# zhaohanjin/hbbft

Hardware: AMD Instinct MI355X
Metric: verified BLS12-381 shares/sec (whole node) at N=1000; combines/sec (higher is better)
Workload: dtype u32 (381-bit Montgomery limbs); 1 GPU; C3 HoneyBadger epoch: 1000 ciphertexts x 1000 DecryptionShares verified + 1000 G1 combines (t=334); N=1000, f=333, t=334, ciphertexts=1000, parallelism=1 GPU

## Files before the change

### hbbft_amd/csrc/curve.h

```cpp
#pragma once
#include "field.h"

namespace hbtc {

HD void fadd(Fq& r, const Fq& a, const Fq& b) { fq_add(r, a, b); }
HD void fadd(Fq2& r, const Fq2& a, const Fq2& b) { fq2_add(r, a, b); }
HD void fsub(Fq& r, const Fq& a, const Fq& b) { fq_sub(r, a, b); }
HD void fsub(Fq2& r, const Fq2& a, const Fq2& b) { fq2_sub(r, a, b); }
HD void fmul(Fq& r, const Fq& a, const Fq& b) { fq_mul(r, a, b); }
HD void fmul(Fq2& r, const Fq2& a, const Fq2& b) { fq2_mul(r, a, b); }
HD void fsqr(Fq& r, const Fq& a) { fq_sqr(r, a); }
HD void fsqr(Fq2& r, const Fq2& a) { fq2_sqr(r, a); }
HD void fdbl(Fq& r, const Fq& a) { fq_dbl(r, a); }
HD void fdbl(Fq2& r, const Fq2& a) { fq2_dbl(r, a); }
HD void fneg(Fq& r, const Fq& a) { fq_neg(r, a); }
HD void fneg(Fq2& r, const Fq2& a) { fq2_neg(r, a); }
HD bool fis_zero(const Fq& a) { return fq_is_zero(a); }
HD bool fis_zero(const Fq2& a) { return fq2_is_zero(a); }
HD bool feq(const Fq& a, const Fq& b) { return fq_eq(a, b); }
HD bool feq(const Fq2& a, const Fq2& b) { return fq2_eq(a, b); }
HD void fone(Fq& r) { fq_one(r); }
HD void fone(Fq2& r) { fq2_one(r); }
HD void fzero(Fq& r) { fq_zero(r); }
HD void fzero(Fq2& r) { fq2_zero(r); }
// ... 1128 lines not shown
    return;
  }
  fw_mul(u1, p.x, z2z2);
  fw_mul(u2, q.x, z1z1);
  fw_mul(s1, p.y, q.z);
  fw_mul(s1, s1, z2z2);
  fw_mul(s2, q.y, p.z);
  fw_mul(s2, s2, z1z1);
  fw_sub(H, u2, u1, rr::RR_SUB_1_4, 4);
  fw_norm(H, H);
  fw_sub(rr0, s2, s1, rr::RR_SUB_1_4, 4);
  fw_norm(rr0, rr0);
  fw_sqr(HH, H);
  if (fw_is_zero(HH)) {
    fw_one(t);
    fw_mul(t, rr0, t);
    if (fw_is_zero(t)) {
      jacw_dbl(r, p);
    } else {
      jacw_set_inf(r);
    }
    return;
  }
  fw_add(t, p.z, q.z);
  fw_norm(t, t);
  fw_sqr(z3, t);
  fw_add(t, z1z1, z2z2);
  fw_sub(z3, z3, t, rr::RR_SUB_2_4, 4);
  fw_norm(z3, z3);
  fw_mul(z3, z3, H);
  jacw_add_tail(r, u1, s1, H, HH, rr0, z3);
}
HD bool jacw_eq_aff(const JacW& p, const FqW& ax, const FqW& ay) {
  FqW z2, z3, t, u, one;
  fw_one(one);
  fw_sqr(z2, p.z);
  fw_mul(z3, z2, p.z);
  fw_mul(t, ax, z2);
  fw_mul(u, p.x, one);
  if (!fw_eq(t, u)) return false;
  fw_mul(t, ay, z3);
  fw_mul(u, p.y, one);
  return fw_eq(t, u);
}
HDN void jacw_mul_x(JacW& r, const AffW& q) {
  JacW acc;
  jacw_set_inf(acc);
  for (int b = 63; b >= 0; --b) {
    jacw_dbl(acc, acc);
    if ((BLS_X_ABS >> b) & 1ull) jacw_add_aff(acc, acc, q);
  }
  r = acc;
}
HDN void jacw_mul_x_jac(JacW& r, const JacW& q) {
  JacW acc;
  jacw_set_inf(acc);
  for (int b = 63; b >= 0; --b) {
    jacw_dbl(acc, acc);
    if ((BLS_X_ABS >> b) & 1ull) jacw_add(acc, acc, q);
  }
  r = acc;
}
HDN bool g1_in_subgroup_t1_w(const G1A& p, G1J& t) {
  if (p.inf) {
    jac_set_inf(t);
    return true;
  }
  AffW q;
  affw_from_aff(q, p);
  JacW t1, t2;
  jacw_mul_x(t1, q);
  jacw_to_jac(t, t1);
  jacw_mul_x_jac(t2, t1);
  if (jacw_is_inf(t2)) return false;
  FqW beta, bx, ny;
  Fq fb;
  fq_set(fb, G1_BETA);
  fw_from_fq(beta, fb);
  fw_mul(bx, q.x, beta);
  fw_neg(ny, q.y);
  return jacw_eq_aff(t2, bx, ny);
}

HD void g2_psi(Fq2& rx, Fq2& ry, const G2A& p) {
  Fq2 c, k;
  fq2_conj(c, p.x);
  fq2_set(k, G2_PSI_CX);
  fq2_mul(rx, c, k);
  fq2_conj(c, p.y);
  fq2_set(k, G2_PSI_CY);
  fq2_mul(ry, c, k);
}

HDN bool g2_in_subgroup(const G2A& p) {
  if (p.inf) return true;
  G2J t;
  jac_mul_u64(t, p, BLS_X_ABS);
  if (jac_is_inf(t)) return false;
  Fq2 px, py, npy;
  g2_psi(px, py, p);
  fq2_neg(npy, py);
  return jac_eq_aff(t, px, npy);
}

HD void g2j_psi(G2J& r, const G2J& p) {
  Fq2 c, k;
  fq2_conj(c, p.x);
  fq2_set(k, G2_PSI_CX);
  fq2_mul(r.x, c, k);
  fq2_conj(c, p.y);
  fq2_set(k, G2_PSI_CY);
  fq2_mul(r.y, c, k);
  fq2_conj(r.z, p.z);
}

HD uint32_t cofactor_c0_word(int i) {
  return i == 0 ? G2_CLEAR_C0[0] : i == 1 ? G2_CLEAR_C0[1] : i == 2 ? G2_CLEAR_C0[2] : G2_CLEAR_C0[3];
}
HDN void g2_clear_cofactor(G2J& out, const G2A& p) {
  if (p.inf) {
    jac_set_inf(out);
    return;
  }
  G2J pj, t1, t2, t3;
  jac_from_aff(pj, p);
  jac_mul_u64(t1, p, BLS_X_ABS);
  jac_neg(t1, t1);
  G2A ps;
  g2_psi(ps.x, ps.y, p);
  ps.inf = 0;
  jac_dbl(t3, pj);
  g2j_psi(t3, t3);
  g2j_psi(t3, t3);
  {
    G2A nps;
    aff_neg(nps, ps);
    jac_add_aff(t3, t3, nps);
  }
  jac_add_aff(t2, t1, ps);
  jac_mul_u64_jac(t2, t2, BLS_X_ABS);
  jac_neg(t2, t2);
  jac_add(t3, t3, t2);
  {
    G2J nt1;
    jac_neg(nt1, t1);
    jac_add(t3, t3, nt1);
  }
  {
    G2A np;
    aff_neg(np, p);
    jac_add_aff(t3, t3, np);
  }
  if (jac_is_inf(t3)) {
    out = t3;
    return;
  }
  G2J mq = t3;
  {
    Fq zeta;
    fq_set(zeta, G2_ZETA);
    fq_mul(mq.x.c0, t3.x.c0, zeta);
    fq_mul(mq.x.c1, t3.x.c1, zeta);
  }
  G2J bj;
  jac_add(bj, t3, mq);
  G2A b;
// ... 184 lines not shown
```

### hbbft_amd/csrc/field.h

```cpp
#pragma once
#include <cstdint>

#if defined(__HIPCC__) || defined(__HIP__)
#include <hip/hip_runtime.h>
#define HD __host__ __device__ __forceinline__
#if defined(HBTC_INLINE_ALL)
#define HDN __host__ __device__ __forceinline__
#else
#define HDN __host__ __device__ inline __attribute__((noinline))
#endif
#define HBTC_CONST static constexpr
#ifndef HBTC_LATENCY_PRIO_LEVEL
#define HBTC_LATENCY_PRIO_LEVEL 2
#endif
#if defined(__HIP_DEVICE_COMPILE__)
#define HBTC_LATENCY_PRIO() __builtin_amdgcn_s_setprio(HBTC_LATENCY_PRIO_LEVEL)
#else
#define HBTC_LATENCY_PRIO() ((void)0)
#endif
#else
#define HD static inline
#define HDN static inline __attribute__((noinline))
#define HBTC_CONST static constexpr
#endif

#include "bls_constants.h"
#include "fq_fips.h"
#ifndef HBTC_FIPS_ONEBLOCK
#define HBTC_FIPS_ONEBLOCK 1
#endif
#if HBTC_FIPS_ONEBLOCK
#include "fq_fips_asm.h"
#endif
#if defined(HBTC_FQMUL_SR)
#include "fq_fips_sr.h"
#endif
#ifndef HBTC_FQ_RR
#define HBTC_FQ_RR 2
#endif
#include "fq_rr.h"

#ifndef HBTC_FQ_UNROLL
#define HBTC_FQ_UNROLL 1
#endif

#define HBTC_PRAGMA(x) _Pragma(#x)
#define HBTC_UNROLL_N(n) HBTC_PRAGMA(unroll n)

namespace hbtc {

template <int N>
struct Limbs {
  uint32_t v[N];
};

typedef Limbs<12> Fq;
typedef Limbs<8> Fr;

HD uint32_t addc32(uint32_t a, uint32_t b, uint32_t cin, uint32_t* cout) {
  return __builtin_addc(a, b, cin, cout);
}
HD uint32_t subb32(uint32_t a, uint32_t b, uint32_t bin, uint32_t* bout) {
  return __builtin_subc(a, b, bin, bout);
}

template <int N>
HD uint32_t limbs_add(Limbs<N>& r, const Limbs<N>& a, const Limbs<N>& b) {
  uint32_t c = 0;
#pragma unroll
  for (int i = 0; i < N; ++i) r.v[i] = addc32(a.v[i], b.v[i], c, &c);
  return c;
}

template <int N>
HD uint32_t limbs_sub(Limbs<N>& r, const Limbs<N>& a, const Limbs<N>& b) {
  uint32_t c = 0;
#pragma unroll
  for (int i = 0; i < N; ++i) r.v[i] = subb32(a.v[i], b.v[i], c, &c);
  return c;
}

template <int N>
HD uint32_t limbs_sub_const(Limbs<N>& r, const Limbs<N>& a, const uint32_t* m) {
  uint32_t c = 0;
#pragma unroll
  for (int i = 0; i < N; ++i) r.v[i] = subb32(a.v[i], m[i], c, &c);
  return c;
}

template <int N>
HD uint32_t limbs_add_const(Limbs<N>& r, const Limbs<N>& a, const uint32_t* m) {
  uint32_t c = 0;
#pragma unroll
  for (int i = 0; i < N; ++i) r.v[i] = addc32(a.v[i], m[i], c, &c);
  return c;
}

template <int N>
HD void limbs_select(Limbs<N>& r, bool take_b, const Limbs<N>& a, const Limbs<N>& b) {
#pragma unroll
  for (int i = 0; i < N; ++i) r.v[i] = take_b ? b.v[i] : a.v[i];
}

template <int N>
HD bool limbs_is_zero(const Limbs<N>& a) {
  uint32_t acc = 0;
#pragma unroll
  for (int i = 0; i < N; ++i) acc |= a.v[i];
  return acc == 0;
}

template <int N>
HD bool limbs_eq(const Limbs<N>& a, const Limbs<N>& b) {
  uint32_t acc = 0;
#pragma unroll
  for (int i = 0; i < N; ++i) acc |= a.v[i] ^ b.v[i];
  return acc == 0;
}

template <int N>
HD bool limbs_lt_const(const Limbs<N>& a, const uint32_t* m) {
// ... 654 lines not shown
}
HD void fw_sqr(FqW& r, const FqW& a) {
#if HBTC_FW_TRACK
  fw_check_operand(a);
  const uint64_t vb = fw_prod_vb(a.vb, a.vb);
#endif
#if defined(__HIP_DEVICE_COMPILE__)
  rr::mont_sqr_w_asm(r.v, a.v);
#else
  rr::mont_sqr_w_cxx(r.v, a.v);
#endif
#if HBTC_FW_TRACK
  fw_set_strict(r, vb);
#endif
}
HD void fw_set(FqW& r, const uint32_t (&c)[13]) {
#pragma unroll
  for (int i = 0; i < 13; ++i) r.v[i] = c[i];
#if HBTC_FW_TRACK
  fw_set_strict(r, FW_ONE_P);
#endif
}
HD void fw_one(FqW& r) { fw_set(r, rr::RR_ONE); }
HD void fw_zero(FqW& r) {
#pragma unroll
  for (int i = 0; i < 13; ++i) r.v[i] = 0;
#if HBTC_FW_TRACK
  uint64_t lb[13] = {0};
  fw_set_bounds(r, lb, 0);
#endif
}
HD void fw_neg(FqW& r, const FqW& a) {
  FqW z;
  fw_zero(z);
  fw_sub(r, z, a, rr::RR_SUB_1_4, 4);
  fw_norm(r, r);
}
HD bool fw_is_zero(const FqW& a) {
#if HBTC_FW_TRACK
  for (int i = 0; i < 12; ++i)
    if (a.lb[i] > rr::RR_MASK) fw_fail("zero test on limbs above 2^30 - 1");
  if (a.vb >= 2 * FW_ONE_P) fw_fail("zero test on a value that may reach 2p");
#endif
  uint32_t z = 0, d = 0;
#pragma unroll
  for (int i = 0; i < 13; ++i) {
    z |= a.v[i];
    d |= a.v[i] ^ rr::RR_P[i];
  }
  return z == 0 || d == 0;
}
HD bool fw_eq(const FqW& a, const FqW& b) {
#if HBTC_FW_TRACK
  for (int i = 0; i < 12; ++i)
    if (a.lb[i] > rr::RR_MASK || b.lb[i] > rr::RR_MASK) fw_fail("comparison on limbs above 2^30 - 1");
  if (a.vb >= 2 * FW_ONE_P || b.vb >= 2 * FW_ONE_P) fw_fail("comparison of a value that may reach 2p");
#endif
  FqR x, y;
#pragma unroll
  for (int i = 0; i < 13; ++i) {
    x.v[i] = a.v[i];
    y.v[i] = b.v[i];
  }
  return fqr_eq(x, y);
}
HD void fw_from_fq(FqW& r, const Fq& a) {
  FqR t;
  fqr_from_fq(t, a);
#pragma unroll
  for (int i = 0; i < 13; ++i) r.v[i] = t.v[i];
#if HBTC_FW_TRACK
  fw_set_strict(r, FW_ONE_P + FW_ONE_P / 2);
#endif
}
HD void fw_to_fq(Fq& r, const FqW& a) {
  FqW k, t;
  fw_set(k, rr::RR_K_OUT);
  fw_mul(t, a, k);
  FqR u;
#pragma unroll
  for (int i = 0; i < 13; ++i) u.v[i] = t.v[i];
  fqr_limbs32(r, u);
}

HD bool fq_is_lex_largest(const Fq& a) {
  Fq c;
  fq_from_mont(c, a);
  Fq t;
  uint32_t borrow = limbs_sub_const<12>(t, c, P_MINUS_1_DIV_2);
  return borrow == 0 && !limbs_is_zero<12>(t);
}

HD void fr_canon(Fr& r, const Fr& a) {
  Fr t;
  uint32_t borrow = limbs_sub_const<8>(t, a, FR_R);
  limbs_select<8>(r, borrow == 0, a, t);
}

HD void fr_mul(Fr& r, const Fr& a, const Fr& b) {
  Fr t;
  mont_mul<8, 8>(t, a, b, FR_R, FR_NP);
  fr_canon(r, t);
}

HD void fr_add(Fr& r, const Fr& a, const Fr& b) {
  limbs_add<8>(r, a, b);
  fr_canon(r, r);
}

HD void fr_sub(Fr& r, const Fr& a, const Fr& b) {
  uint32_t borrow = limbs_sub<8>(r, a, b);
  Fr t;
  limbs_add_const<8>(t, r, FR_R);
  limbs_select<8>(r, borrow != 0, r, t);
}

HD void fr_to_mont(Fr& r, const Fr& a) {
  Fr r2;
  limbs_set_const<8>(r2, FR_R2);
  fr_mul(r, a, r2);
  fr_canon(r, r);
}

HD void fr_from_mont(Fr& r, const Fr& a) {
  Fr one;
  limbs_zero<8>(one);
  one.v[0] = 1;
  fr_mul(r, a, one);
  fr_canon(r, r);
}

HDN void fr_pow_const(Fr& r, const Fr& a, const uint32_t* e) {
  Fr acc;
  limbs_set_const<8>(acc, FR_ONE);
  for (int w = 7; w >= 0; --w) {
    const uint32_t word = e[w];
    for (int b = 31; b >= 0; --b) {
      fr_mul(acc, acc, acc);
      if ((word >> b) & 1u) fr_mul(acc, acc, a);
    }
  }
  fr_canon(r, acc);
}

HD void fr_inv(Fr& r, const Fr& a) { fr_pow_const(r, a, EXP_R_MINUS_2); }

HD void fr_from_u64(Fr& r, uint64_t x) {
  Fr a;
  limbs_zero<8>(a);
  a.v[0] = (uint32_t)x;
  a.v[1] = (uint32_t)(x >> 32);
  fr_to_mont(r, a);
}

struct Fq2 {
  Fq c0, c1;
};

HD void fq2_zero(Fq2& r) {
  fq_zero(r.c0);
  fq_zero(r.c1);
}
HD void fq2_one(Fq2& r) {
  fq_one(r.c0);
  fq_zero(r.c1);
}
// ... 405 lines not shown
```

### hbbft_amd/csrc/fq_rr.h

```cpp
#pragma once
#include <cstdint>
#if defined(__HIPCC__) || defined(__HIP__)
#define HBTC_RR_HD __host__ __device__ __forceinline__
#else
#define HBTC_RR_HD static inline
#endif
#define HBTC_RR_CONST static constexpr
#if defined(HBTC_RR_ASSERT) && !defined(__HIP_DEVICE_COMPILE__)
#include <cstdio>
#include <cstdlib>
#define HBTC_RR_MAD(acc, x, y)                                                          \
  do {                                                                                  \
    if (__builtin_add_overflow((acc), (uint64_t)(x) * (y), &(acc))) {                   \
      std::fprintf(stderr, "fq_rr: MAD carry-out at %s:%d\n", __FILE__, __LINE__);       \
      std::abort();                                                                     \
    }                                                                                   \
  } while (0)
#else
#define HBTC_RR_MAD(acc, x, y) ((acc) += (uint64_t)(x) * (y))
#endif
namespace hbtc {
namespace rr {

HBTC_RR_CONST uint32_t RR_P[13] = {0x3fffaaabu, 0x27fbffffu, 0x153ffffbu, 0x2affffacu, 0x30f6241eu, 0x034a83dau, 0x112bf673u, 0x12e13ce1u, 0x2cd76477u, 0x1ed90d2eu, 0x29a4b1bau, 0x3a8e5ff9u, 0x001a0111u};
// ... 1502 lines not shown
      "v_mad_u64_u32 v[" HBTC_XS(HBTC_FIPS_ACC2) ":" HBTC_XS(HBTC_FIPS_ACC3) "], vcc, %23, %59, v[" HBTC_XS(HBTC_FIPS_ACC2) ":" HBTC_XS(HBTC_FIPS_ACC3) "]\n\t"
      "v_mad_u64_u32 v[" HBTC_XS(HBTC_FIPS_ACC2) ":" HBTC_XS(HBTC_FIPS_ACC3) "], vcc, %24, %58, v[" HBTC_XS(HBTC_FIPS_ACC2) ":" HBTC_XS(HBTC_FIPS_ACC3) "]\n\t"
      "v_mad_u64_u32 v[" HBTC_XS(HBTC_FIPS_ACC2) ":" HBTC_XS(HBTC_FIPS_ACC3) "], vcc, %25, %57, v[" HBTC_XS(HBTC_FIPS_ACC2) ":" HBTC_XS(HBTC_FIPS_ACC3) "]\n\t"
      "v_and_b32 %4, %66, v" HBTC_XS(HBTC_FIPS_ACC2) "\n\t"
      "v_alignbit_b32 v" HBTC_XS(HBTC_FIPS_ACC0) ", v" HBTC_XS(HBTC_FIPS_ACC3) ", v" HBTC_XS(HBTC_FIPS_ACC2) ", 30\n\t"
      "v_lshrrev_b32 v" HBTC_XS(HBTC_FIPS_ACC1) ", 30, v" HBTC_XS(HBTC_FIPS_ACC3) "\n\t"
      "v_mad_u64_u32 v[" HBTC_XS(HBTC_FIPS_ACC0) ":" HBTC_XS(HBTC_FIPS_ACC1) "], vcc, %33, %51, v[" HBTC_XS(HBTC_FIPS_ACC0) ":" HBTC_XS(HBTC_FIPS_ACC1) "]\n\t"
      "v_mad_u64_u32 v[" HBTC_XS(HBTC_FIPS_ACC0) ":" HBTC_XS(HBTC_FIPS_ACC1) "], vcc, %34, %50, v[" HBTC_XS(HBTC_FIPS_ACC0) ":" HBTC_XS(HBTC_FIPS_ACC1) "]\n\t"
      "v_mad_u64_u32 v[" HBTC_XS(HBTC_FIPS_ACC0) ":" HBTC_XS(HBTC_FIPS_ACC1) "], vcc, %35, %49, v[" HBTC_XS(HBTC_FIPS_ACC0) ":" HBTC_XS(HBTC_FIPS_ACC1) "]\n\t"
      "v_mad_u64_u32 v[" HBTC_XS(HBTC_FIPS_ACC0) ":" HBTC_XS(HBTC_FIPS_ACC1) "], vcc, %36, %36, v[" HBTC_XS(HBTC_FIPS_ACC0) ":" HBTC_XS(HBTC_FIPS_ACC1) "]\n\t"
      "v_mad_u64_u32 v[" HBTC_XS(HBTC_FIPS_ACC0) ":" HBTC_XS(HBTC_FIPS_ACC1) "], vcc, %19, %64, v[" HBTC_XS(HBTC_FIPS_ACC0) ":" HBTC_XS(HBTC_FIPS_ACC1) "]\n\t"
      "v_mad_u64_u32 v[" HBTC_XS(HBTC_FIPS_ACC0) ":" HBTC_XS(HBTC_FIPS_ACC1) "], vcc, %20, %63, v[" HBTC_XS(HBTC_FIPS_ACC0) ":" HBTC_XS(HBTC_FIPS_ACC1) "]\n\t"
      "v_mad_u64_u32 v[" HBTC_XS(HBTC_FIPS_ACC0) ":" HBTC_XS(HBTC_FIPS_ACC1) "], vcc, %21, %62, v[" HBTC_XS(HBTC_FIPS_ACC0) ":" HBTC_XS(HBTC_FIPS_ACC1) "]\n\t"
      "v_mad_u64_u32 v[" HBTC_XS(HBTC_FIPS_ACC0) ":" HBTC_XS(HBTC_FIPS_ACC1) "], vcc, %22, %61, v[" HBTC_XS(HBTC_FIPS_ACC0) ":" HBTC_XS(HBTC_FIPS_ACC1) "]\n\t"
      "v_mad_u64_u32 v[" HBTC_XS(HBTC_FIPS_ACC0) ":" HBTC_XS(HBTC_FIPS_ACC1) "], vcc, %23, %60, v[" HBTC_XS(HBTC_FIPS_ACC0) ":" HBTC_XS(HBTC_FIPS_ACC1) "]\n\t"
      "v_mad_u64_u32 v[" HBTC_XS(HBTC_FIPS_ACC0) ":" HBTC_XS(HBTC_FIPS_ACC1) "], vcc, %24, %59, v[" HBTC_XS(HBTC_FIPS_ACC0) ":" HBTC_XS(HBTC_FIPS_ACC1) "]\n\t"
      "v_mad_u64_u32 v[" HBTC_XS(HBTC_FIPS_ACC0) ":" HBTC_XS(HBTC_FIPS_ACC1) "], vcc, %25, %58, v[" HBTC_XS(HBTC_FIPS_ACC0) ":" HBTC_XS(HBTC_FIPS_ACC1) "]\n\t"
      "v_and_b32 %5, %66, v" HBTC_XS(HBTC_FIPS_ACC0) "\n\t"
      "v_alignbit_b32 v" HBTC_XS(HBTC_FIPS_ACC2) ", v" HBTC_XS(HBTC_FIPS_ACC1) ", v" HBTC_XS(HBTC_FIPS_ACC0) ", 30\n\t"
      "v_lshrrev_b32 v" HBTC_XS(HBTC_FIPS_ACC3) ", 30, v" HBTC_XS(HBTC_FIPS_ACC1) "\n\t"
      "v_mad_u64_u32 v[" HBTC_XS(HBTC_FIPS_ACC2) ":" HBTC_XS(HBTC_FIPS_ACC3) "], vcc, %34, %51, v[" HBTC_XS(HBTC_FIPS_ACC2) ":" HBTC_XS(HBTC_FIPS_ACC3) "]\n\t"
      "v_mad_u64_u32 v[" HBTC_XS(HBTC_FIPS_ACC2) ":" HBTC_XS(HBTC_FIPS_ACC3) "], vcc, %35, %50, v[" HBTC_XS(HBTC_FIPS_ACC2) ":" HBTC_XS(HBTC_FIPS_ACC3) "]\n\t"
      "v_mad_u64_u32 v[" HBTC_XS(HBTC_FIPS_ACC2) ":" HBTC_XS(HBTC_FIPS_ACC3) "], vcc, %36, %49, v[" HBTC_XS(HBTC_FIPS_ACC2) ":" HBTC_XS(HBTC_FIPS_ACC3) "]\n\t"
      "v_mad_u64_u32 v[" HBTC_XS(HBTC_FIPS_ACC2) ":" HBTC_XS(HBTC_FIPS_ACC3) "], vcc, %20, %64, v[" HBTC_XS(HBTC_FIPS_ACC2) ":" HBTC_XS(HBTC_FIPS_ACC3) "]\n\t"
      "v_mad_u64_u32 v[" HBTC_XS(HBTC_FIPS_ACC2) ":" HBTC_XS(HBTC_FIPS_ACC3) "], vcc, %21, %63, v[" HBTC_XS(HBTC_FIPS_ACC2) ":" HBTC_XS(HBTC_FIPS_ACC3) "]\n\t"
      "v_mad_u64_u32 v[" HBTC_XS(HBTC_FIPS_ACC2) ":" HBTC_XS(HBTC_FIPS_ACC3) "], vcc, %22, %62, v[" HBTC_XS(HBTC_FIPS_ACC2) ":" HBTC_XS(HBTC_FIPS_ACC3) "]\n\t"
      "v_mad_u64_u32 v[" HBTC_XS(HBTC_FIPS_ACC2) ":" HBTC_XS(HBTC_FIPS_ACC3) "], vcc, %23, %61, v[" HBTC_XS(HBTC_FIPS_ACC2) ":" HBTC_XS(HBTC_FIPS_ACC3) "]\n\t"
      "v_mad_u64_u32 v[" HBTC_XS(HBTC_FIPS_ACC2) ":" HBTC_XS(HBTC_FIPS_ACC3) "], vcc, %24, %60, v[" HBTC_XS(HBTC_FIPS_ACC2) ":" HBTC_XS(HBTC_FIPS_ACC3) "]\n\t"
      "v_mad_u64_u32 v[" HBTC_XS(HBTC_FIPS_ACC2) ":" HBTC_XS(HBTC_FIPS_ACC3) "], vcc, %25, %59, v[" HBTC_XS(HBTC_FIPS_ACC2) ":" HBTC_XS(HBTC_FIPS_ACC3) "]\n\t"
      "v_and_b32 %6, %66, v" HBTC_XS(HBTC_FIPS_ACC2) "\n\t"
      "v_alignbit_b32 v" HBTC_XS(HBTC_FIPS_ACC0) ", v" HBTC_XS(HBTC_FIPS_ACC3) ", v" HBTC_XS(HBTC_FIPS_ACC2) ", 30\n\t"
      "v_lshrrev_b32 v" HBTC_XS(HBTC_FIPS_ACC1) ", 30, v" HBTC_XS(HBTC_FIPS_ACC3) "\n\t"
      "v_mad_u64_u32 v[" HBTC_XS(HBTC_FIPS_ACC0) ":" HBTC_XS(HBTC_FIPS_ACC1) "], vcc, %35, %51, v[" HBTC_XS(HBTC_FIPS_ACC0) ":" HBTC_XS(HBTC_FIPS_ACC1) "]\n\t"
      "v_mad_u64_u32 v[" HBTC_XS(HBTC_FIPS_ACC0) ":" HBTC_XS(HBTC_FIPS_ACC1) "], vcc, %36, %50, v[" HBTC_XS(HBTC_FIPS_ACC0) ":" HBTC_XS(HBTC_FIPS_ACC1) "]\n\t"
      "v_mad_u64_u32 v[" HBTC_XS(HBTC_FIPS_ACC0) ":" HBTC_XS(HBTC_FIPS_ACC1) "], vcc, %37, %37, v[" HBTC_XS(HBTC_FIPS_ACC0) ":" HBTC_XS(HBTC_FIPS_ACC1) "]\n\t"
      "v_mad_u64_u32 v[" HBTC_XS(HBTC_FIPS_ACC0) ":" HBTC_XS(HBTC_FIPS_ACC1) "], vcc, %21, %64, v[" HBTC_XS(HBTC_FIPS_ACC0) ":" HBTC_XS(HBTC_FIPS_ACC1) "]\n\t"
      "v_mad_u64_u32 v[" HBTC_XS(HBTC_FIPS_ACC0) ":" HBTC_XS(HBTC_FIPS_ACC1) "], vcc, %22, %63, v[" HBTC_XS(HBTC_FIPS_ACC0) ":" HBTC_XS(HBTC_FIPS_ACC1) "]\n\t"
      "v_mad_u64_u32 v[" HBTC_XS(HBTC_FIPS_ACC0) ":" HBTC_XS(HBTC_FIPS_ACC1) "], vcc, %23, %62, v[" HBTC_XS(HBTC_FIPS_ACC0) ":" HBTC_XS(HBTC_FIPS_ACC1) "]\n\t"
      "v_mad_u64_u32 v[" HBTC_XS(HBTC_FIPS_ACC0) ":" HBTC_XS(HBTC_FIPS_ACC1) "], vcc, %24, %61, v[" HBTC_XS(HBTC_FIPS_ACC0) ":" HBTC_XS(HBTC_FIPS_ACC1) "]\n\t"
      "v_mad_u64_u32 v[" HBTC_XS(HBTC_FIPS_ACC0) ":" HBTC_XS(HBTC_FIPS_ACC1) "], vcc, %25, %60, v[" HBTC_XS(HBTC_FIPS_ACC0) ":" HBTC_XS(HBTC_FIPS_ACC1) "]\n\t"
      "v_and_b32 %7, %66, v" HBTC_XS(HBTC_FIPS_ACC0) "\n\t"
      "v_alignbit_b32 v" HBTC_XS(HBTC_FIPS_ACC2) ", v" HBTC_XS(HBTC_FIPS_ACC1) ", v" HBTC_XS(HBTC_FIPS_ACC0) ", 30\n\t"
      "v_lshrrev_b32 v" HBTC_XS(HBTC_FIPS_ACC3) ", 30, v" HBTC_XS(HBTC_FIPS_ACC1) "\n\t"
      "v_mad_u64_u32 v[" HBTC_XS(HBTC_FIPS_ACC2) ":" HBTC_XS(HBTC_FIPS_ACC3) "], vcc, %36, %51, v[" HBTC_XS(HBTC_FIPS_ACC2) ":" HBTC_XS(HBTC_FIPS_ACC3) "]\n\t"
      "v_mad_u64_u32 v[" HBTC_XS(HBTC_FIPS_ACC2) ":" HBTC_XS(HBTC_FIPS_ACC3) "], vcc, %37, %50, v[" HBTC_XS(HBTC_FIPS_ACC2) ":" HBTC_XS(HBTC_FIPS_ACC3) "]\n\t"
      "v_mad_u64_u32 v[" HBTC_XS(HBTC_FIPS_ACC2) ":" HBTC_XS(HBTC_FIPS_ACC3) "], vcc, %22, %64, v[" HBTC_XS(HBTC_FIPS_ACC2) ":" HBTC_XS(HBTC_FIPS_ACC3) "]\n\t"
      "v_mad_u64_u32 v[" HBTC_XS(HBTC_FIPS_ACC2) ":" HBTC_XS(HBTC_FIPS_ACC3) "], vcc, %23, %63, v[" HBTC_XS(HBTC_FIPS_ACC2) ":" HBTC_XS(HBTC_FIPS_ACC3) "]\n\t"
      "v_mad_u64_u32 v[" HBTC_XS(HBTC_FIPS_ACC2) ":" HBTC_XS(HBTC_FIPS_ACC3) "], vcc, %24, %62, v[" HBTC_XS(HBTC_FIPS_ACC2) ":" HBTC_XS(HBTC_FIPS_ACC3) "]\n\t"
      "v_mad_u64_u32 v[" HBTC_XS(HBTC_FIPS_ACC2) ":" HBTC_XS(HBTC_FIPS_ACC3) "], vcc, %25, %61, v[" HBTC_XS(HBTC_FIPS_ACC2) ":" HBTC_XS(HBTC_FIPS_ACC3) "]\n\t"
      "v_and_b32 %8, %66, v" HBTC_XS(HBTC_FIPS_ACC2) "\n\t"
      "v_alignbit_b32 v" HBTC_XS(HBTC_FIPS_ACC0) ", v" HBTC_XS(HBTC_FIPS_ACC3) ", v" HBTC_XS(HBTC_FIPS_ACC2) ", 30\n\t"
      "v_lshrrev_b32 v" HBTC_XS(HBTC_FIPS_ACC1) ", 30, v" HBTC_XS(HBTC_FIPS_ACC3) "\n\t"
      "v_mad_u64_u32 v[" HBTC_XS(HBTC_FIPS_ACC0) ":" HBTC_XS(HBTC_FIPS_ACC1) "], vcc, %37, %51, v[" HBTC_XS(HBTC_FIPS_ACC0) ":" HBTC_XS(HBTC_FIPS_ACC1) "]\n\t"
      "v_mad_u64_u32 v[" HBTC_XS(HBTC_FIPS_ACC0) ":" HBTC_XS(HBTC_FIPS_ACC1) "], vcc, %38, %38, v[" HBTC_XS(HBTC_FIPS_ACC0) ":" HBTC_XS(HBTC_FIPS_ACC1) "]\n\t"
      "v_mad_u64_u32 v[" HBTC_XS(HBTC_FIPS_ACC0) ":" HBTC_XS(HBTC_FIPS_ACC1) "], vcc, %23, %64, v[" HBTC_XS(HBTC_FIPS_ACC0) ":" HBTC_XS(HBTC_FIPS_ACC1) "]\n\t"
      "v_mad_u64_u32 v[" HBTC_XS(HBTC_FIPS_ACC0) ":" HBTC_XS(HBTC_FIPS_ACC1) "], vcc, %24, %63, v[" HBTC_XS(HBTC_FIPS_ACC0) ":" HBTC_XS(HBTC_FIPS_ACC1) "]\n\t"
      "v_mad_u64_u32 v[" HBTC_XS(HBTC_FIPS_ACC0) ":" HBTC_XS(HBTC_FIPS_ACC1) "], vcc, %25, %62, v[" HBTC_XS(HBTC_FIPS_ACC0) ":" HBTC_XS(HBTC_FIPS_ACC1) "]\n\t"
      "v_and_b32 %9, %66, v" HBTC_XS(HBTC_FIPS_ACC0) "\n\t"
      "v_alignbit_b32 v" HBTC_XS(HBTC_FIPS_ACC2) ", v" HBTC_XS(HBTC_FIPS_ACC1) ", v" HBTC_XS(HBTC_FIPS_ACC0) ", 30\n\t"
      "v_lshrrev_b32 v" HBTC_XS(HBTC_FIPS_ACC3) ", 30, v" HBTC_XS(HBTC_FIPS_ACC1) "\n\t"
      "v_mad_u64_u32 v[" HBTC_XS(HBTC_FIPS_ACC2) ":" HBTC_XS(HBTC_FIPS_ACC3) "], vcc, %38, %51, v[" HBTC_XS(HBTC_FIPS_ACC2) ":" HBTC_XS(HBTC_FIPS_ACC3) "]\n\t"
      "v_mad_u64_u32 v[" HBTC_XS(HBTC_FIPS_ACC2) ":" HBTC_XS(HBTC_FIPS_ACC3) "], vcc, %24, %64, v[" HBTC_XS(HBTC_FIPS_ACC2) ":" HBTC_XS(HBTC_FIPS_ACC3) "]\n\t"
      "v_mad_u64_u32 v[" HBTC_XS(HBTC_FIPS_ACC2) ":" HBTC_XS(HBTC_FIPS_ACC3) "], vcc, %25, %63, v[" HBTC_XS(HBTC_FIPS_ACC2) ":" HBTC_XS(HBTC_FIPS_ACC3) "]\n\t"
      "v_and_b32 %10, %66, v" HBTC_XS(HBTC_FIPS_ACC2) "\n\t"
      "v_alignbit_b32 v" HBTC_XS(HBTC_FIPS_ACC0) ", v" HBTC_XS(HBTC_FIPS_ACC3) ", v" HBTC_XS(HBTC_FIPS_ACC2) ", 30\n\t"
      "v_lshrrev_b32 v" HBTC_XS(HBTC_FIPS_ACC1) ", 30, v" HBTC_XS(HBTC_FIPS_ACC3) "\n\t"
      "v_mad_u64_u32 v[" HBTC_XS(HBTC_FIPS_ACC0) ":" HBTC_XS(HBTC_FIPS_ACC1) "], vcc, %39, %39, v[" HBTC_XS(HBTC_FIPS_ACC0) ":" HBTC_XS(HBTC_FIPS_ACC1) "]\n\t"
      "v_mad_u64_u32 v[" HBTC_XS(HBTC_FIPS_ACC0) ":" HBTC_XS(HBTC_FIPS_ACC1) "], vcc, %25, %64, v[" HBTC_XS(HBTC_FIPS_ACC0) ":" HBTC_XS(HBTC_FIPS_ACC1) "]\n\t"
      "v_and_b32 %11, %66, v" HBTC_XS(HBTC_FIPS_ACC0) "\n\t"
      "v_alignbit_b32 %12, v" HBTC_XS(HBTC_FIPS_ACC1) ", v" HBTC_XS(HBTC_FIPS_ACC0) ", 30\n\t"
      : "=&v"(r[0]), "=&v"(r[1]), "=&v"(r[2]), "=&v"(r[3]), "=&v"(r[4]), "=&v"(r[5]), "=&v"(r[6]), "=&v"(r[7]), "=&v"(r[8]), "=&v"(r[9]), "=&v"(r[10]), "=&v"(r[11]), "=&v"(r[12]),
        "=&v"(q[0]), "=&v"(q[1]), "=&v"(q[2]), "=&v"(q[3]), "=&v"(q[4]), "=&v"(q[5]), "=&v"(q[6]), "=&v"(q[7]), "=&v"(q[8]), "=&v"(q[9]), "=&v"(q[10]), "=&v"(q[11]), "=&v"(q[12]), "=&v"(h)
      : "v"(a[0]), "v"(a[1]), "v"(a[2]), "v"(a[3]), "v"(a[4]), "v"(a[5]), "v"(a[6]), "v"(a[7]), "v"(a[8]), "v"(a[9]), "v"(a[10]), "v"(a[11]), "v"(a[12]),
        "v"(d[1]), "v"(d[2]), "v"(d[3]), "v"(d[4]), "v"(d[5]), "v"(d[6]), "v"(d[7]), "v"(d[8]), "v"(d[9]), "v"(d[10]), "v"(d[11]), "v"(d[12]),
        "s"(RR_P[0]), "s"(RR_P[1]), "s"(RR_P[2]), "s"(RR_P[3]), "s"(RR_P[4]), "s"(RR_P[5]), "s"(RR_P[6]), "s"(RR_P[7]), "s"(RR_P[8]), "s"(RR_P[9]), "s"(RR_P[10]), "s"(RR_P[11]), "s"(RR_P[12]), "s"(RR_NP), "s"(RR_MASK)
      : "v" HBTC_XS(HBTC_FIPS_ACC0), "v" HBTC_XS(HBTC_FIPS_ACC1), "v" HBTC_XS(HBTC_FIPS_ACC2), "v" HBTC_XS(HBTC_FIPS_ACC3), "vcc");
}

#endif

HBTC_RR_CONST uint32_t RR_W_SLACK = 3u;
HBTC_RR_CONST uint32_t RR_W_TOP = 0x0680447au;
HBTC_RR_CONST uint32_t RR_ONE[13] = {0x00d1ff2eu, 0x19d80000u, 0x34800ac4u, 0x2e00cde6u, 0x02431c84u, 0x269f83a2u, 0x3dcf80ddu, 0x09b42da0u, 0x25eec26cu, 0x15d98f12u, 0x04b29f14u, 0x259fcfa0u, 0x00015de9u};
HBTC_RR_CONST uint32_t RR_SUB_1_4[13] = {0x7ffeaaacu, 0x5feffffeu, 0x54ffffedu, 0x6bfffeb0u, 0x43d89079u, 0x4d2a0f6au, 0x44afd9cbu, 0x4b84f384u, 0x735d91dcu, 0x7b6434b9u, 0x6692c6e8u, 0x6a397fe5u, 0x00680446u};
HBTC_RR_CONST uint32_t RR_SUB_2_4[13] = {0xbffeaaacu, 0x9feffffdu, 0x94ffffecu, 0xabfffeafu, 0x83d89078u, 0x8d2a0f69u, 0x84afd9cau, 0x8b84f383u, 0xb35d91dbu, 0xbb6434b8u, 0xa692c6e7u, 0xaa397fe4u, 0x00680445u};
HBTC_RR_CONST uint32_t RR_SUB_2_8[13] = {0xbffd5558u, 0xbfdffffdu, 0xa9ffffdau, 0x97fffd60u, 0x87b120f3u, 0x9a541ed4u, 0x895fb396u, 0x9709e708u, 0xa6bb23b8u, 0xb6c86973u, 0x8d258dd1u, 0x9472ffcbu, 0x00d0088du};
HBTC_RR_CONST uint32_t RR_SUB_2_10[13] = {0xbffcaaaeu, 0x8fd7fffdu, 0x947fffd2u, 0xadfffcb9u, 0xa99d6930u, 0xa0e92689u, 0xabb7a07cu, 0xbccc60cau, 0x8069eca6u, 0xb47a83d1u, 0xa06ef146u, 0x898fbfbeu, 0x01040ab1u};
HBTC_RR_CONST uint32_t RR_SUB_2_14[13] = {0xbffb555au, 0xafc7fffdu, 0xa97fffc0u, 0x99fffb6au, 0xad75f9abu, 0xae1335f4u, 0xb0677a48u, 0x8851544fu, 0xb3c77e84u, 0xafdeb88bu, 0x8701b830u, 0xb3c93fa5u, 0x016c0ef8u};

HBTC_RR_HD void mont_mul_w_cxx(uint32_t* r, const uint32_t* a, const uint32_t* b) {
  const uint32_t* p = RR_P;
  uint32_t q[13], t[13], h = 0;
  uint64_t acc;
  acc = (uint64_t)a[0] * b[0];
  q[0] = ((uint32_t)acc * RR_NP) & RR_MASK;
  HBTC_RR_MAD(acc, q[0], p[0]);
  acc >>= 30;
  HBTC_RR_MAD(acc, a[0], b[1]);
  HBTC_RR_MAD(acc, a[1], b[0]);
  HBTC_RR_MAD(acc, q[0], p[1]);
  q[1] = ((uint32_t)acc * RR_NP) & RR_MASK;
  HBTC_RR_MAD(acc, q[1], p[0]);
  acc >>= 30;
  HBTC_RR_MAD(acc, a[0], b[2]);
  HBTC_RR_MAD(acc, a[1], b[1]);
  HBTC_RR_MAD(acc, a[2], b[0]);
  HBTC_RR_MAD(acc, q[0], p[2]);
  HBTC_RR_MAD(acc, q[1], p[1]);
  q[2] = ((uint32_t)acc * RR_NP) & RR_MASK;
  HBTC_RR_MAD(acc, q[2], p[0]);
  acc >>= 30;
  HBTC_RR_MAD(acc, a[0], b[3]);
  HBTC_RR_MAD(acc, a[1], b[2]);
  HBTC_RR_MAD(acc, a[2], b[1]);
  HBTC_RR_MAD(acc, a[3], b[0]);
  HBTC_RR_MAD(acc, q[0], p[3]);
  HBTC_RR_MAD(acc, q[1], p[2]);
  HBTC_RR_MAD(acc, q[2], p[1]);
  q[3] = ((uint32_t)acc * RR_NP) & RR_MASK;
  HBTC_RR_MAD(acc, q[3], p[0]);
  acc >>= 30;
  HBTC_RR_MAD(acc, a[0], b[4]);
  HBTC_RR_MAD(acc, a[1], b[3]);
  HBTC_RR_MAD(acc, a[2], b[2]);
  HBTC_RR_MAD(acc, a[3], b[1]);
  HBTC_RR_MAD(acc, a[4], b[0]);
  HBTC_RR_MAD(acc, q[0], p[4]);
  HBTC_RR_MAD(acc, q[1], p[3]);
  HBTC_RR_MAD(acc, q[2], p[2]);
  HBTC_RR_MAD(acc, q[3], p[1]);
  q[4] = ((uint32_t)acc * RR_NP) & RR_MASK;
  HBTC_RR_MAD(acc, q[4], p[0]);
  acc >>= 30;
  HBTC_RR_MAD(acc, a[0], b[5]);
  HBTC_RR_MAD(acc, a[1], b[4]);
  HBTC_RR_MAD(acc, a[2], b[3]);
  HBTC_RR_MAD(acc, a[3], b[2]);
  HBTC_RR_MAD(acc, a[4], b[1]);
  HBTC_RR_MAD(acc, a[5], b[0]);
  HBTC_RR_MAD(acc, q[0], p[5]);
  HBTC_RR_MAD(acc, q[1], p[4]);
  HBTC_RR_MAD(acc, q[2], p[3]);
  HBTC_RR_MAD(acc, q[3], p[2]);
  HBTC_RR_MAD(acc, q[4], p[1]);
  q[5] = ((uint32_t)acc * RR_NP) & RR_MASK;
  HBTC_RR_MAD(acc, q[5], p[0]);
  acc >>= 30;
  HBTC_RR_MAD(acc, a[0], b[6]);
  HBTC_RR_MAD(acc, a[1], b[5]);
  HBTC_RR_MAD(acc, a[2], b[4]);
  HBTC_RR_MAD(acc, a[3], b[3]);
  HBTC_RR_MAD(acc, a[4], b[2]);
  HBTC_RR_MAD(acc, a[5], b[1]);
  HBTC_RR_MAD(acc, a[6], b[0]);
  HBTC_RR_MAD(acc, q[0], p[6]);
  HBTC_RR_MAD(acc, q[1], p[5]);
  HBTC_RR_MAD(acc, q[2], p[4]);
  HBTC_RR_MAD(acc, q[3], p[3]);
  HBTC_RR_MAD(acc, q[4], p[2]);
  HBTC_RR_MAD(acc, q[5], p[1]);
  q[6] = ((uint32_t)acc * RR_NP) & RR_MASK;
  HBTC_RR_MAD(acc, q[6], p[0]);
  acc >>= 30;
  HBTC_RR_MAD(acc, a[0], b[7]);
  HBTC_RR_MAD(acc, a[1], b[6]);
  HBTC_RR_MAD(acc, a[2], b[5]);
// ... 1471 lines not shown
```

### hbbft_amd/csrc/hbtc_rlc.hip

```cpp
#include "rlc_common.h"
#include "rlc_tree.h"

#ifndef HBTC_PART
#define HBTC_PART 0
#endif
#define HBTC_IN_PART(n) (HBTC_PART == 0 || HBTC_PART == (n))

#ifndef HBTC_RLC_SPLIT
#define HBTC_RLC_SPLIT 1
#endif
#ifndef HBTC_RLC_TREE
#define HBTC_RLC_TREE 1
#endif
#if HBTC_RLC_TREE && !HBTC_RLC_SPLIT
#error "HBTC_RLC_TREE needs HBTC_RLC_SPLIT (S_i is left in the t1 workspace)"
#endif
#ifndef HBTC_TREE_WAVES
#define HBTC_TREE_WAVES 2
#endif
#ifndef HBTC_TREE_PRIO
#define HBTC_TREE_PRIO 0
#endif

namespace hbtc {
// ... 88 lines not shown
  const uint32_t id = blockIdx.x * 64u + threadIdx.x;
  if (id >= n_pk) return;
  G1J r;
  rlc_sender_point(r, id, pk, pk_status, pk_tab, key);
  rpk[id] = r;
}

__global__ void __launch_bounds__(64, HBTC_ITEMS_WAVES) k_rlc_items(
    const Tile* __restrict__ tiles, const uint32_t* __restrict__ idx,
    const uint8_t* __restrict__ shares, const int32_t* __restrict__ pk_status, uint32_t n_pk,
    RlcKey key, Suspects sus, TileSums* __restrict__ sums, G1A* __restrict__ dec,
    int32_t* __restrict__ status, G1J* __restrict__ t1s, const G1J* __restrict__ rpk,
    uint64_t* __restrict__ masks) {
#if HBTC_ITEMS_PRIO > 0
  __builtin_amdgcn_s_setprio(HBTC_ITEMS_PRIO);
#endif
  __shared__ G1J red[128];
  const Tile tile = tiles[blockIdx.x];
  const uint32_t lane = threadIdx.x;
  const size_t item = (size_t)tile.first + lane;
  G1J S;
  jac_set_inf(S);
#if !HBTC_RLC_TREE
  G1J P;
  jac_set_inf(P);
#endif
  int32_t st = HBTC_RLC_PENDING;
  uint32_t id = 0;
  bool sum = false;
#if !HBTC_RLC_SPLIT
  G1A d;
  G1J t1;
#endif
  if (lane < tile.count) {
    id = idx[item];
    if (id >= n_pk) {
      st = HBTC_UNKNOWN_SENDER;
    } else if (pk_status[id] != HBTC_ACCEPT) {
      st = HBTC_DECODE_ERR;
    } else {
#if HBTC_RLC_SPLIT
      const bool dec_ok = status[item] != HBTC_DECODE_ERR;
#else
      uint32_t w[12];
      rlc_load_words(w, shares, item, 12);
      const bool dec_ok = g1_decompress_t1(d, t1, w);
      if (dec_ok) dec[item] = d;
#endif
      if (!dec_ok) {
        st = HBTC_DECODE_ERR;
      } else if (is_suspect(sus, id)) {
        st = HBTC_RLC_LEAF;
      } else {
        sum = true;
      }
    }
  }
  {
    const uint32_t mine = sum ? id : 0xffffffffu;
    bool dup = false;
#pragma unroll 1
    for (uint32_t j = 0; j < 63; ++j) {
      const uint32_t other = (uint32_t)__shfl((int)mine, (int)j);
      dup |= j < lane && other == mine;
    }
    if (sum && dup) {
      sum = false;
      st = HBTC_RLC_LEAF;
    }
  }
  if (lane < tile.count) status[item] = st;
  rlc_list_leaf(sus, st == HBTC_RLC_LEAF, (uint32_t)item, tile.inst, lane);
  if (sum) {
#if HBTC_RLC_SPLIT
    const G1A d = dec[item];
    G1J t1 = t1s[item];
#endif
    if (!d.inf) {
      const XDigits xd = rlc_digits(key, id);
      jac_neg(t1, t1);
      Fq beta;
      fq_set(beta, G1_BETA);
#if HBTC_XADIC8
#if HBTC_ITEMS_WAVES >= 2 && HBTC_SAC8_LDS
      xadic_mul_sac8<Fq, true>(S, d, t1, beta, xd.d[0], xd.d[1], xd.d[2], xd.d[3], xd.nbits,
                               reinterpret_cast<uint32_t*>(red), lane);
#else
      xadic_mul_sac8(S, d, t1, beta, xd.d[0], xd.d[1], xd.d[2], xd.d[3], xd.nbits);
#endif
#else
      G1A xp, pxp;
      xadic_table(xp, pxp, d, t1);
      xadic_mul_uniform(S, d, xp, pxp, beta, xd.d[0], xd.d[1], xd.d[2], xd.d[3], xd.nbits);
#endif
    }
#if !HBTC_RLC_TREE
    P = rpk[id];
#endif
  }
#if HBTC_RLC_TREE
  if (lane < tile.count) t1s[item] = S;
  const uint64_t m = __ballot(sum);
  if (lane == 0) masks[blockIdx.x] = m;
#else
  G1J* redA = red;
  G1J* redB = red + 64;
  TileSums* ts = sums + blockIdx.x;
  rlc_reduce_sp(redA, redB, S, P, lane, ts->S, ts->SW, ts->P, ts->PW, ts->SH, ts->SHW, ts->PH,
                ts->PHW, ts->SQ, ts->SQW, ts->PQ, ts->PQW);
#endif
}

#endif

#if HBTC_IN_PART(6)
__global__ void __launch_bounds__(64) k_rlc_finalize(const Tile* __restrict__ tiles,
                                                     const int32_t* __restrict__ h_status,
                                                     const int32_t* __restrict__ w_status,
                                                     int32_t* __restrict__ status,
                                                     const uint32_t* __restrict__ idx, uint32_t n_pk,
                                                     uint32_t* __restrict__ rejects) {
  const Tile tile = tiles[blockIdx.x];
  if (threadIdx.x >= tile.count) return;
  const uint32_t i = tile.first + threadIdx.x;
  if (h_status[tile.inst] != HBTC_ACCEPT || w_status[tile.inst] != HBTC_ACCEPT) {
    status[i] = HBTC_INSTANCE_ERR;
  } else {
    const int32_t st = status[i];
    if (st == HBTC_RLC_PENDING) {
      status[i] = HBTC_ACCEPT;
    } else if (st == HBTC_REJECT && rejects) {
      const uint32_t id = idx[i];
      if (id < n_pk) atomicAdd(rejects + id, 1u);
    }
  }
}

__global__ void __launch_bounds__(256) k_status_remap(uint32_t n, int32_t* __restrict__ status,
                                                      int32_t from, int32_t to) {
  const uint32_t i = blockIdx.x * blockDim.x + threadIdx.x;
  if (i < n && status[i] == from) status[i] = to;
}

__global__ void __launch_bounds__(256) k_track_update(uint32_t n_pk, uint32_t* __restrict__ rejects,
                                                      uint32_t* __restrict__ last_bad, uint32_t now,
                                                      uint32_t thresh) {
  const uint32_t i = blockIdx.x * blockDim.x + threadIdx.x;
  if (i >= n_pk) return;
  const uint32_t r = rejects[i];
  if (r == 0) return;
  if (r >= thresh) last_bad[i] = now;
  rejects[i] = 0;
}
#endif

#if HBTC_IN_PART(7) && HBTC_RLC_TREE
static_assert(sizeof(TileSums) == TS_G1J * sizeof(G1J) && offsetof(TileSums, P) == TS_P * sizeof(G1J) &&
                  offsetof(TileSums, SW) == TS_SW * sizeof(G1J) && offsetof(TileSums, PW) == TS_PW * sizeof(G1J) &&
                  offsetof(TileSums, SH) == TS_SH * sizeof(G1J) && offsetof(TileSums, SHW) == TS_SHW * sizeof(G1J) &&
                  offsetof(TileSums, PH) == TS_PH * sizeof(G1J) && offsetof(TileSums, PHW) == TS_PHW * sizeof(G1J) &&
                  offsetof(TileSums, SQ) == TS_SQ * sizeof(G1J) && offsetof(TileSums, SQW) == TS_SQW * sizeof(G1J) &&
                  offsetof(TileSums, PQ) == TS_PQ * sizeof(G1J) && offsetof(TileSums, PQW) == TS_PQW * sizeof(G1J),
              "rlc_tree.h addresses TileSums as an array of G1J");
__global__ void __launch_bounds__(TREE_BS, HBTC_TREE_WAVES) k_rlc_tree(
    uint32_t n_tiles, const Tile* __restrict__ tiles, const uint32_t* __restrict__ idx,
    const uint64_t* __restrict__ masks, G1J* t1s, G1J* pnodes, const G1J* __restrict__ rpk,
    TileSums* sums) {
// ... 84 lines not shown
```

Measured before the change: 18.67 million shares/s.

## Add wide-limb co-Z table build and SAC8 multiply path for RLC items

Adds a 30-bit-limb (FqW) version of the 8-entry x-adic SAC table construction, built from co-Z additions with lazy rescaling of earlier entries, plus a main loop that uses wide-limb doubling and mixed addition. The RLC item kernel is switched to this path when HBTC_FQ_RR>=3, and the default HBTC_FQ_RR is raised from 2 to 3. The aim is to cut field-multiply cost through the redundant-limb arithmetic and to avoid per-entry inversions when building the table. In exchange it adds pack/unpack conversions on every table access, and the default bump may also change other code paths gated on HBTC_FQ_RR.

```diff
diff --git a/hbbft_amd/csrc/curve.h b/hbbft_amd/csrc/curve.h
--- a/hbbft_amd/csrc/curve.h
+++ b/hbbft_amd/csrc/curve.h
@@ -1234,6 +1234,233 @@
   return jacw_eq_aff(t2, bx, ny);
 }
 
+struct XYW {
+  FqW x, y;
+};
+HD void jacw_madd_generic(JacW& r, const JacW& p, const FqW& qx, const FqW& qy) {
+  FqW z1z1, u2, s2, H, HH, rr0, z3;
+  fw_sqr(z1z1, p.z);
+  fw_mul(u2, qx, z1z1);
+  fw_mul(s2, qy, p.z);
+  fw_mul(s2, s2, z1z1);
+  fw_sub(H, u2, p.x, rr::RR_SUB_2_14, 14);
+  fw_norm(H, H);
+  fw_sub(rr0, s2, p.y, rr::RR_SUB_2_14, 14);
+  fw_norm(rr0, rr0);
+  fw_sqr(HH, H);
+  fw_mul(z3, p.z, H);
+  fw_dbl(z3, z3);
+  fw_norm(z3, z3);
+  jacw_add_tail(r, p.x, p.y, H, HH, rr0, z3);
+}
+HD void coz_add_w(XYW& s, FqW& ax, FqW& ay, FqW& h, const XYW& b) {
+  FqW r, hh, hhh, v, t, one;
+  fw_sub(h, b.x, ax, rr::RR_SUB_1_4, 4);
+  fw_norm(h, h);
+  fw_sub(r, b.y, ay, rr::RR_SUB_1_4, 4);
+  fw_norm(r, r);
+  fw_sqr(hh, h);
+  fw_mul(hhh, hh, h);
+  fw_mul(v, ax, hh);
+  fw_mul(ay, ay, hhh);
+  ax = v;
+  fw_sqr(t, r);
+  fw_sub(t, t, hhh, rr::RR_SUB_1_4, 4);
+  fw_norm(t, t);
+  fw_dbl(hh, v);
+  fw_sub(t, t, hh, rr::RR_SUB_2_4, 4);
+  fw_norm(t, t);
+  fw_one(one);
+  fw_mul(s.x, t, one);
+  fw_sub(t, v, t, rr::RR_SUB_2_10, 10);
+  fw_norm(t, t);
+  fw_mul(t, r, t);
+  fw_sub(t, t, ay, rr::RR_SUB_1_4, 4);
+  fw_norm(t, t);
+  fw_mul(s.y, t, one);
+}
+HD void xyw_pack(XY<Fq>& r, const XYW& a) {
+  fw_pack(r.x, a.x);
+  fw_pack(r.y, a.y);
+}
+HD void xyw_unpack(XYW& r, const XY<Fq>& a) {
+  fw_unpack(r.x, a.x);
+  fw_unpack(r.y, a.y);
+}
+HD void xyw_rescale(XY<Fq>& p, const FqW& h2, const FqW& h3) {
+  FqW t;
+  fw_unpack(t, p.x);
+  fw_mul(t, t, h2);
+  fw_pack(p.x, t);
+  fw_unpack(t, p.y);
+  fw_mul(t, t, h3);
+  fw_pack(p.y, t);
+}
+HD void xyw_lds_rescale(uint32_t* lds, uint32_t lane, int e, const FqW& h2, const FqW& h3) {
+  XY<Fq> v;
+  xy_lds_get(v, lds, lane, e);
+  xyw_rescale(v, h2, h3);
+  xy_lds_put(lds, lane, e, v);
+}
+HD void xadic_table8_chain_w(XY<Fq> tab[5], Fq& zsp, const G1A& p, const G1J& xpj, uint32_t* lds, uint32_t lane) {
+  XY<Fq>& P = tab[0];
+  XY<Fq>& S = tab[1];
+  XY<Fq> X;
+  FqW h, h2, h3, zs;
+  {
+    FqW z, z2, z3;
+    XYW pw, xw, sw;
+    fw_from_fq(z, xpj.z);
+    fw_sqr(z2, z);
+    fw_mul(z3, z2, z);
+    fw_from_fq(pw.x, p.x);
+    fw_mul(pw.x, pw.x, z2);
+    fw_from_fq(pw.y, p.y);
+    fw_mul(pw.y, pw.y, z3);
+    fw_from_fq(xw.x, xpj.x);
+    fw_from_fq(xw.y, xpj.y);
+    coz_add_w(sw, xw.x, xw.y, h, pw);
+    xyw_pack(S, sw);
+    xyw_pack(X, xw);
+    fw_sqr(h2, h);
+    fw_mul(h3, h2, h);
+    fw_mul(pw.x, pw.x, h2);
+    fw_mul(pw.y, pw.y, h3);
+    xyw_pack(P, pw);
+    fw_mul(zs, z, h);
+  }
+  auto sum = [&](XY<Fq>& out, XY<Fq>& U, const XY<Fq>& V) {
+    XYW mv, u, o;
+    FqW beta;
+    fw_set(beta, rr::RR_BETA);
+    fw_unpack(mv.x, V.x);
+    fw_mul(mv.x, mv.x, beta);
+    fw_unpack(mv.y, V.y);
+    xyw_unpack(u, U);
+    coz_add_w(o, u.x, u.y, h, mv);
+    xyw_pack(out, o);
+    xyw_pack(U, u);
+    fw_sqr(h2, h);
+    fw_mul(h3, h2, h);
+    fw_mul(zs, zs, h);
+  };
+  sum(tab[4], P, X);
+  xyw_rescale(X, h2, h3);
+  xyw_rescale(S, h2, h3);
+  {
+    XY<Fq> t5;
+    sum(t5, S, X);
+    xy_lds_put(lds, lane, 0, t5);
+  }
+  xyw_rescale(P, h2, h3);
+  xyw_rescale(tab[4], h2, h3);
+  sum(tab[2], P, P);
+  xyw_rescale(S, h2, h3);
+  xyw_rescale(tab[4], h2, h3);
+  xyw_lds_rescale(lds, lane, 0, h2, h3);
+  sum(tab[3], S, P);
+  xyw_rescale(P, h2, h3);
+  xyw_rescale(tab[2], h2, h3);
+  xyw_rescale(tab[4], h2, h3);
+  xyw_lds_rescale(lds, lane, 0, h2, h3);
+  {
+    XY<Fq> t6;
+    sum(t6, P, S);
+    xy_lds_put(lds, lane, 1, t6);
+  }
+  xyw_rescale(S, h2, h3);
+  xyw_rescale(tab[2], h2, h3);
+  xyw_rescale(tab[3], h2, h3);
+  xyw_rescale(tab[4], h2, h3);
+  xyw_lds_rescale(lds, lane, 0, h2, h3);
+  {
+    XY<Fq> t7;
+    const XY<Fq> s0 = S;
+    sum(t7, S, s0);
+    xy_lds_put(lds, lane, 2, t7);
+  }
+  xyw_rescale(P, h2, h3);
+  xyw_rescale(tab[2], h2, h3);
+  xyw_rescale(tab[3], h2, h3);
+  xyw_rescale(tab[4], h2, h3);
+  xyw_lds_rescale(lds, lane, 0, h2, h3);
+  xyw_lds_rescale(lds, lane, 1, h2, h3);
+  fw_pack(zsp, zs);
+}
+HD void xadic_mul_sac8_w(G1J& r, const G1A& p, const G1J& xpj, uint32_t d0, uint32_t d1, uint32_t d2,
+                         uint32_t d3, int nbits, uint32_t* lds, uint32_t lane) {
+  constexpr int NWD = 24;
+  XY<Fq> tab[5];
+  Fq zsp;
+  xadic_table8_chain_w(tab, zsp, p, xpj, lds, lane);
+  const uint32_t k0 = d0 | 1u;
+  uint64_t m[3];
+  xadic_sac_recode(m, k0, d1, d2, d3, nbits);
+  auto entry = [&](int i, XYW& t) {
+    const bool b1 = ((m[0] >> i) & 1u) != 0, b2 = ((m[1] >> i) & 1u) != 0;
+    const bool b3 = ((m[2] >> i) & 1u) != 0;
+    XY<Fq> e0, e1, e;
+    {
+      XY<Fq> a, b;
+      xy_sel(a, b1, tab[1], tab[0]);
+      xy_sel(b, b1, tab[3], tab[2]);
+      xy_sel(e0, b2, b, a);
+    }
+    {
+      const uint32_t j = (b1 ? 1u : 0u) + (b2 ? 2u : 0u);
+      const uint32_t li = j ? j - 1u : 0u;
+      XY<Fq> l;
+      uint32_t* dst = reinterpret_cast<uint32_t*>(&l);
+#pragma unroll
+      for (int w = 0; w < NWD; ++w) dst[w] = lds[(li * NWD + w) * 64 + lane];
+      xy_sel(e1, j != 0, l, tab[4]);
+    }
+    xy_sel(e, b3, e1, e0);
+    xyw_unpack(t, e);
+    const bool neg = i < nbits && (((uint64_t)k0 >> (i + 1)) & 1u) == 0;
+    FqW ny;
+    fw_neg(ny, t.y);
+    fw_sel(t.y, neg, ny, t.y);
+  };
+  JacW acc;
+  {
+    XYW t;
+    entry(nbits, t);
+    acc.x = t.x;
+    acc.y = t.y;
+    fw_one(acc.z);
+  }
+#pragma unroll 1
+  for (int i = nbits - 1; i >= 0; --i) {
+    jacw_dbl(acc, acc);
+    XYW t;
+    entry(i, t);
+    jacw_madd_generic(acc, acc, t.x, t.y);
+  }
+  {
+    const bool even = (d0 & 1u) == 0;
+    const bool zero = (d0 | d1 | d2 | d3) == 0;
+    XYW t;
+    xyw_unpack(t, tab[0]);
+    FqW ny;
+    fw_neg(ny, t.y);
+    JacW n;
+    jacw_madd_generic(n, acc, t.x, ny);
+    fw_sel(acc.x, even, n.x, acc.x);
+    fw_sel(acc.y, even, n.y, acc.y);
+    fw_sel(acc.z, even, n.z, acc.z);
+    FqW z0;
+    fw_zero(z0);
+    fw_sel(acc.z, zero, z0, acc.z);
+  }
+  {
+    FqW zs;
+    fw_unpack(zs, zsp);
+    fw_mul(acc.z, acc.z, zs);
+  }
+  jacw_to_jac(r, acc);
+}
+
 HD void g2_psi(Fq2& rx, Fq2& ry, const G2A& p) {
   Fq2 c, k;
   fq2_conj(c, p.x);
diff --git a/hbbft_amd/csrc/field.h b/hbbft_amd/csrc/field.h
--- a/hbbft_amd/csrc/field.h
+++ b/hbbft_amd/csrc/field.h
@@ -36,7 +36,7 @@
 #include "fq_fips_sr.h"
 #endif
 #ifndef HBTC_FQ_RR
-#define HBTC_FQ_RR 2
+#define HBTC_FQ_RR 3
 #endif
 #include "fq_rr.h"
 
@@ -857,6 +857,38 @@
   for (int i = 0; i < 13; ++i) u.v[i] = t.v[i];
   fqr_limbs32(r, u);
 }
+HD void fw_sel(FqW& r, bool c, const FqW& a, const FqW& b) {
+#if HBTC_FW_TRACK
+  uint64_t lb[13];
+  for (int i = 0; i < 13; ++i) lb[i] = a.lb[i] > b.lb[i] ? a.lb[i] : b.lb[i];
+  const uint64_t vb = a.vb > b.vb ? a.vb : b.vb;
+#endif
+#pragma unroll
+  for (int i = 0; i < 13; ++i) r.v[i] = c ? a.v[i] : b.v[i];
+#if HBTC_FW_TRACK
+  fw_set_bounds(r, lb, vb);
+#endif
+}
+HD void fw_pack(Fq& r, const FqW& a) {
+#if HBTC_FW_TRACK
+  for (int i = 0; i < 13; ++i)
+    if (a.lb[i] > rr::RR_MASK) fw_fail("packing limbs above 2^30 - 1");
+  if (a.vb > FW_ONE_P + FW_ONE_P / 2) fw_fail("packing a value that may pass 1.5p");
+#endif
+  FqR t;
+#pragma unroll
+  for (int i = 0; i < 13; ++i) t.v[i] = a.v[i];
+  fqr_limbs32(r, t);
+}
+HD void fw_unpack(FqW& r, const Fq& a) {
+  FqR t;
+  fqr_limbs30(t, a);
+#pragma unroll
+  for (int i = 0; i < 13; ++i) r.v[i] = t.v[i];
+#if HBTC_FW_TRACK
+  fw_set_strict(r, FW_ONE_P + FW_ONE_P / 2);
+#endif
+}
 
 HD bool fq_is_lex_largest(const Fq& a) {
   Fq c;
diff --git a/hbbft_amd/csrc/fq_rr.h b/hbbft_amd/csrc/fq_rr.h
--- a/hbbft_amd/csrc/fq_rr.h
+++ b/hbbft_amd/csrc/fq_rr.h
@@ -1608,6 +1608,7 @@
 HBTC_RR_CONST uint32_t RR_W_SLACK = 3u;
 HBTC_RR_CONST uint32_t RR_W_TOP = 0x0680447au;
 HBTC_RR_CONST uint32_t RR_ONE[13] = {0x00d1ff2eu, 0x19d80000u, 0x34800ac4u, 0x2e00cde6u, 0x02431c84u, 0x269f83a2u, 0x3dcf80ddu, 0x09b42da0u, 0x25eec26cu, 0x15d98f12u, 0x04b29f14u, 0x259fcfa0u, 0x00015de9u};
+HBTC_RR_CONST uint32_t RR_BETA[13] = {0x229d39fcu, 0x11661b79u, 0x3a68a8f8u, 0x09dabbd8u, 0x12744b7eu, 0x22bc97d4u, 0x3c5ccd3eu, 0x1cf87540u, 0x0197e4f4u, 0x3433d1ecu, 0x0d20861fu, 0x33953662u, 0x000edc53u};
 HBTC_RR_CONST uint32_t RR_SUB_1_4[13] = {0x7ffeaaacu, 0x5feffffeu, 0x54ffffedu, 0x6bfffeb0u, 0x43d89079u, 0x4d2a0f6au, 0x44afd9cbu, 0x4b84f384u, 0x735d91dcu, 0x7b6434b9u, 0x6692c6e8u, 0x6a397fe5u, 0x00680446u};
 HBTC_RR_CONST uint32_t RR_SUB_2_4[13] = {0xbffeaaacu, 0x9feffffdu, 0x94ffffecu, 0xabfffeafu, 0x83d89078u, 0x8d2a0f69u, 0x84afd9cau, 0x8b84f383u, 0xb35d91dbu, 0xbb6434b8u, 0xa692c6e7u, 0xaa397fe4u, 0x00680445u};
 HBTC_RR_CONST uint32_t RR_SUB_2_8[13] = {0xbffd5558u, 0xbfdffffdu, 0xa9ffffdau, 0x97fffd60u, 0x87b120f3u, 0x9a541ed4u, 0x895fb396u, 0x9709e708u, 0xa6bb23b8u, 0xb6c86973u, 0x8d258dd1u, 0x9472ffcbu, 0x00d0088du};
diff --git a/hbbft_amd/csrc/hbtc_rlc.hip b/hbbft_amd/csrc/hbtc_rlc.hip
--- a/hbbft_amd/csrc/hbtc_rlc.hip
+++ b/hbbft_amd/csrc/hbtc_rlc.hip
@@ -194,7 +194,11 @@
       Fq beta;
       fq_set(beta, G1_BETA);
 #if HBTC_XADIC8
-#if HBTC_ITEMS_WAVES >= 2 && HBTC_SAC8_LDS
+#if HBTC_ITEMS_WAVES >= 2 && HBTC_SAC8_LDS && HBTC_FQ_RR >= 3 && HBTC_RLC_SPLIT && HBTC_RLC_TREE
+      (void)beta;
+      xadic_mul_sac8_w(S, d, t1, xd.d[0], xd.d[1], xd.d[2], xd.d[3], xd.nbits,
+                       reinterpret_cast<uint32_t*>(red), lane);
+#elif HBTC_ITEMS_WAVES >= 2 && HBTC_SAC8_LDS
       xadic_mul_sac8<Fq, true>(S, d, t1, beta, xd.d[0], xd.d[1], xd.d[2], xd.d[3], xd.nbits,
                                reinterpret_cast<uint32_t*>(red), lane);
 #else
```

After: 19.81 million shares/s, median of 6. 6.1% higher.
